# payakorn/InteriorPointMethod

Measured on AMD Instinct MI355X. Metric: IPM iterations/sec (m=4096,n=8192 dense LP), higher is better.
Workload: dtype f64; 1 GPU; dense synthetic LP m=4096 n=8192 fp64, seed 0, start x=s=1 y=0 (BASELINE.json configs[1]); replicas per GPU

## Files before the change

interiorpointmethod_amd/csrc/ff_schedule.h:

```cpp
#pragma once
#include <stdint.h>
#include <stdio.h>
#include <stdlib.h>

#include <math.h>

#include <algorithm>
#include <limits>
#include <queue>
#include <set>
#include <string>
#include <vector>

namespace ipm {

struct FFItem {
    unsigned char type;
    unsigned char i, c;
    unsigned char q;
    union {
        struct { unsigned char j0, j1, flags, seq; } t;
        struct { unsigned short s0, s1; } f;
    };
};
enum { FF_F = 0, FF_T = 1, FF_D = 2 };
enum { FF_INIT = 1, FF_ADD_BASE = 2, FF_PANEL = 4, FF_SIG_DIAG = 8 };
constexpr int FF_MAX_NBLK = 96;

#if defined(__HIPCC__)
#define FF_HD __host__ __device__
#else
#define FF_HD
#endif
FF_HD inline int ff_tile(int i, int c) { return i * (i + 1) / 2 + c; }

struct FFWords {
    static constexpr unsigned ticket = 0;
    static constexpr unsigned role = 3;
    static constexpr unsigned maxbits = 8;
    static constexpr unsigned dcount = 10;
    static constexpr unsigned dbg = 24;
    static constexpr unsigned dbg_end = 32;
    static constexpr unsigned fcount = 32;
    size_t tprog;
    size_t lfinal;
    size_t dready;
    size_t potrfdone;
    size_t count;
    FF_HD explicit FFWords(int nblk) {
        const size_t ntile = (size_t)nblk * ((size_t)nblk + 1) / 2;
        tprog = fcount + ntile; lfinal = tprog + ntile; dready = lfinal + (size_t)nblk; potrfdone = dready + (size_t)nblk;
        count = potrfdone + (size_t)nblk;
    }
    FF_HD static const unsigned* base_of_dbg(const unsigned* dbg_words) { return dbg_words - dbg; }
};

struct FFModel {
    double f_over = 6.1, f_stage = 4.02;
    double f_stage_half = 2.1;
    double t_over = 7.0, t_col = 15.9;
    double t_rmw = 1.0, t_panel = 18.3;
    double t_base = 2.3;
    double d_item = 130.0;
    double gap = 0.8, handoff = 1.0;
    double potrf = 36.8, cpanel = 7.3, cupdate = 7.3;
    int batch = 4;
    int tail = 2;
    double stagger = 0.3;
    int nstages = 512;
    int q_last = 0;
};

struct FFSchedule {
    std::vector<FFItem> items;
    std::vector<int> tile_items;
    std::vector<int> tile_q;
    double makespan_us = 0.0;
    double form_end_us = 0.0;
};

inline int ff_limit(int i, int c) { return (i == c) ? (c > 0 ? c - 1 : 0) : c; }
inline bool ff_needs_panel(int i, int c) { return i > c + 1; }

inline void ff_build_schedule(int nblk, int Q, int W, const FFModel& M_in, FFSchedule& out, int Qmax = 0) {
    if (Qmax < Q) Qmax = Q;
    const double INF = std::numeric_limits<double>::infinity();
    const int ntile = nblk * (nblk + 1) / 2;
    FFModel Mx = M_in;
    if (const char* e = getenv("IPM_FF_BATCH")) Mx.batch = std::max(1, atoi(e));
    if (const char* e = getenv("IPM_FF_TAIL")) Mx.tail = std::max(1, atoi(e));
    if (const char* e = getenv("IPM_FF_STAGGER")) Mx.stagger = std::min(0.9, std::max(0.0, atof(e)));
    if (const char* e = getenv("IPM_FF_Q_LAST")) Mx.q_last = std::max(0, atoi(e));
    if (const char* e = getenv("IPM_FF_MODEL")) {
        std::string spec(e);
        size_t p0 = 0;
        while (p0 < spec.size()) {
            size_t p1 = spec.find(',', p0); if (p1 == std::string::npos) p1 = spec.size();
            const std::string kv = spec.substr(p0, p1 - p0);
            const size_t eq = kv.find('=');
            if (eq != std::string::npos) {
                const std::string k = kv.substr(0, eq); const double v = atof(kv.c_str() + eq + 1);
                struct { const char* n; double* p; } tab[] = {{"f_over", &Mx.f_over}, {"f_stage", &Mx.f_stage}, {"f_stage_half", &Mx.f_stage_half}, {"t_over", &Mx.t_over}, {"t_col", &Mx.t_col},
                    {"t_rmw", &Mx.t_rmw}, {"t_panel", &Mx.t_panel}, {"t_base", &Mx.t_base}, {"d_item", &Mx.d_item}, {"potrf", &Mx.potrf},
                    {"cpanel", &Mx.cpanel}, {"cupdate", &Mx.cupdate}, {"handoff", &Mx.handoff}, {"gap", &Mx.gap}};
                for (auto& t : tab) if (k == t.n) *t.p = v;
            }
            p0 = p1 + 1;
        }
    }
    const FFModel& M = Mx;
    enum Kind { K_F, K_T, K_D, K_POTRF, K_CPANEL, K_CUPDATE };
    struct Node {
        Kind kind; int i = 0, c = 0, q = 0, j0 = 0, j1 = 0, flags = 0, seq = 0, s0 = 0, s1 = 0;
        double dur = 0.0, bl = 0.0, est = 0.0, fin = 0.0;
        int npred = 0, left = 0;
        std::vector<int> succ;
    };
    std::vector<Node> nd;
    nd.reserve((size_t)ntile * 6 + 4 * (size_t)nblk);
    auto add = [&](Kind k, double dur) { Node x; x.kind = k; x.dur = dur; x.fin = INF; nd.push_back(x); return (int)nd.size() - 1; };
    auto edge = [&](int a, int b) { nd[(size_t)a].succ.push_back(b); nd[(size_t)b].npred++; };
    std::vector<int> potrf((size_t)nblk), cpan, cupd;
    for (int k = 0; k < nblk; ++k) { potrf[(size_t)k] = add(K_POTRF, M.potrf + M.handoff); nd.back().i = k; }
    cpan.resize((size_t)nblk - 1); cupd.resize((size_t)nblk - 1);
    for (int k = 0; k + 1 < nblk; ++k) { cpan[(size_t)k] = add(K_CPANEL, M.cpanel + M.handoff); nd.back().i = k; }
    for (int k = 0; k + 1 < nblk; ++k) { cupd[(size_t)k] = add(K_CUPDATE, M.cupdate + M.handoff); nd.back().i = k; }
    for (int k = 0; k + 1 < nblk; ++k) { edge(potrf[(size_t)k], cpan[(size_t)k]); edge(cpan[(size_t)k], cupd[(size_t)k]); edge(cupd[(size_t)k], potrf[(size_t)k + 1]); }
    std::vector<std::vector<int>> titems((size_t)ntile);
    std::vector<int> lprod((size_t)ntile, -1);
    for (int i = 0; i < nblk; ++i)
        for (int c = 0; c <= i; ++c) {
            const int lim = ff_limit(i, c);
            const bool pan = ff_needs_panel(i, c);
            std::vector<std::pair<int, int>> cuts;
            const int nb_end = std::max(0, lim - M.tail);
            int j = 0;
            while (j + M.batch <= nb_end) { cuts.emplace_back(j, j + M.batch); j += M.batch; }
            if (j < nb_end) { cuts.emplace_back(j, nb_end); j = nb_end; }
            while (j < lim) { cuts.emplace_back(j, j + 1); ++j; }
            if (cuts.empty()) cuts.emplace_back(0, 0);
            std::vector<int>& ids = titems[(size_t)ff_tile(i, c)];
            for (size_t s = 0; s < cuts.size(); ++s) {
                const bool last = s + 1 == cuts.size();
                const int id = add(K_T, M.t_over + M.t_col * (cuts[s].second - cuts[s].first) + (s ? M.t_rmw : 0.0) + ((last && pan) ? M.t_panel : 0.0) + M.handoff + M.gap);
                Node& x = nd[(size_t)id];
                x.i = i; x.c = c; x.j0 = cuts[s].first; x.j1 = cuts[s].second; x.seq = (int)s + 1;
                x.flags = (s == 0 ? FF_INIT : 0) | ((last && pan) ? FF_PANEL : 0) | ((last && i == 0 && c == 0) ? FF_SIG_DIAG : 0);
                if (s) edge(ids.back(), id);
                ids.push_back(id);
            }
            if (pan) lprod[(size_t)ff_tile(i, c)] = ids.back();
        }
    for (int k = 0; k + 1 < nblk; ++k) {
        lprod[(size_t)ff_tile(k + 1, k)] = cpan[(size_t)k];
        edge(titems[(size_t)ff_tile(k + 1, k)].back(), cpan[(size_t)k]);
        edge(titems[(size_t)ff_tile(k + 1, k + 1)].back(), cupd[(size_t)k]);
    }
    edge(titems[0].back(), potrf[0]);
    for (int t = 0; t < ntile; ++t)
        for (int id : titems[(size_t)t]) {
            const int i = nd[(size_t)id].i, c = nd[(size_t)id].c, j1 = nd[(size_t)id].j1;
            if (j1 > nd[(size_t)id].j0) {
                edge(lprod[(size_t)ff_tile(i, j1 - 1)], id);
                if (c != i) edge(lprod[(size_t)ff_tile(c, j1 - 1)], id);
            }
            if (nd[(size_t)id].flags & FF_PANEL) edge(potrf[(size_t)c], id);
        }
    std::vector<int> base_item((size_t)ntile);
    for (int t = 0; t < ntile; ++t) { const std::vector<int>& ids = titems[(size_t)t]; base_item[(size_t)t] = ids.size() == 1 ? ids[0] : ids[ids.size() - 2]; }
    std::vector<int> fch;
    out.tile_q.assign((size_t)ntile, 0);
    {
        int npairs = 0;
        for (int i = 0; i < nblk; i += 2)
            for (int c = 0; c <= std::min(i + 1, nblk - 1); ++c) {
                int q = (M.q_last > 0 && i + 2 >= nblk) ? M.q_last : Q;
                q = std::max(1, std::min(std::min(q, Qmax), M.nstages));
                const double phi = std::fmod(npairs * 0.381966, 1.0);
                ++npairs;
                std::vector<int> cut((size_t)q + 1, 0);
                double tot = 0.0, acc = 0.0;
                std::vector<double> len((size_t)q);
                for (int k = 0; k < q; ++k) { len[(size_t)k] = 1.0 + M.stagger * (2.0 * std::fmod((double)k / q + phi, 1.0) - 1.0); tot += len[(size_t)k]; }
                for (int k = 0; k < q; ++k) { acc += len[(size_t)k]; cut[(size_t)k + 1] = (int)(M.nstages * acc / tot + 0.5); }
                cut[(size_t)q] = M.nstages;
                for (int k = 0; k < q; ++k) {
                    const bool half = c > i || i + 1 >= nblk;
                    const int id = add(K_F, M.f_over + (half ? M.f_stage_half : M.f_stage) * (cut[(size_t)k + 1] - cut[(size_t)k]) + M.gap);
                    Node& x = nd[(size_t)id];
                    x.i = i; x.c = c; x.q = k; x.s0 = cut[(size_t)k]; x.s1 = cut[(size_t)k + 1];
                    fch.push_back(id);
                    for (int r = i; r <= i + 1; ++r)
                        if (r >= c && r < nblk) { edge(id, base_item[(size_t)ff_tile(r, c)]); out.tile_q[(size_t)ff_tile(r, c)]++; }
                }
            }
    }
    for (int t = 0; t < ntile; ++t) { Node& x = nd[(size_t)base_item[(size_t)t]]; x.flags |= FF_ADD_BASE; x.dur += M.t_base * out.tile_q[(size_t)t]; }
    std::vector<int> ditems;
    for (int i = 0; i < nblk; ++i) { const int id = add(K_D, M.d_item + M.gap); nd[(size_t)id].i = i; edge(id, potrf[0]); ditems.push_back(id); }
    const int N = (int)nd.size();
    {
        std::vector<int> order, indeg((size_t)N), stack;
        order.reserve((size_t)N);
        for (int u = 0; u < N; ++u) { indeg[(size_t)u] = nd[(size_t)u].npred; if (!indeg[(size_t)u]) stack.push_back(u); }
        while (!stack.empty()) {
            const int u = stack.back(); stack.pop_back(); order.push_back(u);
            for (int v : nd[(size_t)u].succ) if (--indeg[(size_t)v] == 0) stack.push_back(v);
        }
        if ((int)order.size() != N) { out.items.clear(); return; }
        for (size_t k = order.size(); k-- > 0;) {
            Node& x = nd[(size_t)order[k]];
            double b = 0.0;
            for (int v : x.succ) b = std::max(b, nd[(size_t)v].bl);
            x.bl = x.dur + b;
        }
    }
    typedef std::pair<double, int> PI;
    std::priority_queue<PI, std::vector<PI>, std::greater<PI>> avail_F;
    std::set<PI> avail_T;
    for (int id : fch) avail_F.push(PI(-nd[(size_t)id].bl, id));
    for (int u = 0; u < N; ++u) nd[(size_t)u].left = nd[(size_t)u].npred;
    std::vector<int> rel;
    auto release = [&](int u0) {
        rel.clear(); rel.push_back(u0);
        while (!rel.empty()) {
            const int u = rel.back(); rel.pop_back();
            for (int v : nd[(size_t)u].succ) {
                Node& y = nd[(size_t)v];
                y.est = std::max(y.est, nd[(size_t)u].fin);
                if (--y.left == 0) {
                    if (y.kind == K_T) avail_T.insert(PI(-y.bl, v));
                    else if (y.kind != K_F && y.kind != K_D) {
                        y.fin = y.est + y.dur;
                        rel.push_back(v);
                    }
                }
            }
        }
    };
    for (int t = 0; t < ntile; ++t) { const int id = titems[(size_t)t][0]; if (nd[(size_t)id].left == 0) avail_T.insert(PI(-nd[(size_t)id].bl, id)); }
    typedef std::pair<double, int> Ev;
    std::priority_queue<Ev, std::vector<Ev>, std::greater<Ev>> free_at;
    for (int w = 0; w < W; ++w) free_at.push(Ev(0.0, w));
    out.items.clear();
    size_t nT = 0, doneT = 0, nextD = 0;
    for (int t = 0; t < ntile; ++t) nT += titems[(size_t)t].size();
    std::vector<int> order_out;
    int guard = 0;
    while (doneT < nT || !avail_F.empty() || nextD < ditems.size()) {
        const Ev ev = free_at.top(); free_at.pop();
        const double t = ev.first;
        if (nextD < ditems.size()) {
            const int v = ditems[nextD++];
            nd[(size_t)v].fin = t + nd[(size_t)v].dur;
            order_out.push_back(v); release(v);
            free_at.push(Ev(nd[(size_t)v].fin, ev.second));
            continue;
        }
        int pick = -1;
        for (const PI& p : avail_T) if (nd[(size_t)p.second].est <= t) { pick = p.second; break; }
        if (pick >= 0 && !avail_F.empty() && -avail_F.top().first > nd[(size_t)pick].bl) pick = -1;
        if (pick < 0 && !avail_F.empty()) {
            const int v = avail_F.top().second; avail_F.pop();
            nd[(size_t)v].fin = t + nd[(size_t)v].dur;
            out.form_end_us = std::max(out.form_end_us, nd[(size_t)v].fin);
            order_out.push_back(v); release(v);
            free_at.push(Ev(nd[(size_t)v].fin, ev.second));
            continue;
        }
        if (pick < 0) {
            if (avail_T.empty()) {
                if (++guard > 64 * W * nblk) break;
                free_at.push(Ev(t + 5.0, ev.second));
                continue;
            }
            double best = INF;
            for (const PI& p : avail_T) if (nd[(size_t)p.second].est < best) { best = nd[(size_t)p.second].est; pick = p.second; }
        }
        Node& x = nd[(size_t)pick];
        avail_T.erase(PI(-x.bl, pick));
        x.fin = std::max(t, x.est) + x.dur;
        order_out.push_back(pick); ++doneT;
        release(pick);
        free_at.push(Ev(x.fin, ev.second));
    }
    out.tile_items.assign((size_t)ntile, 0);
    for (int t = 0; t < ntile; ++t) out.tile_items[(size_t)t] = (int)titems[(size_t)t].size();
    out.makespan_us = 0.0;
    for (int v : order_out) {
        const Node& x = nd[(size_t)v];
        FFItem it{};
        it.i = (unsigned char)x.i; it.c = (unsigned char)x.c;
        if (x.kind == K_F) { it.type = FF_F; it.q = (unsigned char)x.q; it.f.s0 = (unsigned short)x.s0; it.f.s1 = (unsigned short)x.s1; }
        else if (x.kind == K_D) { it.type = FF_D; }
        else { it.type = FF_T; it.t.j0 = (unsigned char)x.j0; it.t.j1 = (unsigned char)x.j1; it.t.flags = (unsigned char)x.flags; it.t.seq = (unsigned char)x.seq; }
        out.items.push_back(it);
    }
    for (int k = 0; k < nblk; ++k) out.makespan_us = std::max(out.makespan_us, nd[(size_t)potrf[(size_t)k]].fin);
}

}
```

interiorpointmethod_amd/csrc/form_factor.h:

```cpp
#pragma once
#include <hip/hip_runtime.h>
#include <stdint.h>

#include "ff_schedule.h"
#include "gemm_nt_f64.h"
#include "handoff.h"
#include "potrf_f64.h"

namespace ipm {

constexpr int FF_THREADS = 512;
constexpr int FF_BK = 32, FF_LDT = FF_BK + 2;
constexpr int FF_OP = 128 * FF_LDT;
constexpr int FF_LDS_DOUBLES = 4 * FF_OP;

struct FFArgs {
    const double* A; int64_t lda;
    const double* d;
    double* B; int64_t ldb;
    const double* invD;
    double* slab;
    const FFItem* items; int nitems;
    unsigned* ticket;
    unsigned* fcount;
    unsigned* tprog;
    unsigned* lfinal;
    unsigned* dready;
    const unsigned* potrfdone;
    unsigned* timeout;
    unsigned* dbg;
    unsigned dbg_words;
    long long* prof;
    long long* trace;
    const int* done;
    int nblk, Q, nstages;
    int m;
    const int* tile_q;
    unsigned long long* maxbits;
    unsigned* dcount;
};

__device__ __forceinline__ void ff_wait_ge(const unsigned* p, unsigned v, unsigned* timeout, unsigned* dbg = nullptr, unsigned item = 0,
                                           unsigned kind = 0, unsigned nw = 0) {
    (void)handoff_wait<2, false>([=] { return handoff_load(p) >= v; }, {timeout, dbg}, [=] {
        handoff_record_ge(dbg, item, kind, v, p);
        const unsigned* live = FFWords::base_of_dbg(dbg);
        unsigned* snap = const_cast<unsigned*>(live) + nw;
        for (unsigned w = 0; w < nw; ++w) snap[w] = handoff_load(live + w);
    });
}

constexpr int FF_BASE_DEPTH = 4;

template <bool SCALE, bool SRC_REGS>
__device__ __forceinline__ void ff_gemm(const double* __restrict__ Pg, int64_t ldp, const double* __restrict__ Qg, int64_t ldq,
                                        const double* __restrict__ w, int ns, double* lds, f64x4 (&acc)[4][2],
                                        const f64x4 (*src)[2]) {
    const int tid = threadIdx.x, lane = tid & 63;
    const int wave = __builtin_amdgcn_readfirstlane(tid >> 6);
    const int wm = wave >> 2, wn = wave & 3;
    const int fr = lane & 15, fk = lane >> 4;
    double* Ps = lds;
    double* Qs = lds + 2 * FF_OP;
    const int ch = tid & 15, r0 = tid >> 4;
    const double* pP = SRC_REGS ? nullptr : Pg + (int64_t)r0 * ldp + ch * 2;
    const double* pQ = Qg + (int64_t)r0 * ldq + ch * 2;
    f64x2 pr[4], qr[4], wr;
    auto load_stage = [&](int s) {
        if (SCALE) wr = *reinterpret_cast<const f64x2*>(w + (int64_t)s * FF_BK + ch * 2);
#pragma unroll
        for (int u = 0; u < 4; ++u) qr[u] = *reinterpret_cast<const f64x2*>(pQ + (int64_t)u * 32 * ldq + (int64_t)s * FF_BK);
        if (!SRC_REGS) {
#pragma unroll
            for (int u = 0; u < 4; ++u) pr[u] = *reinterpret_cast<const f64x2*>(pP + (int64_t)u * 32 * ldp + (int64_t)s * FF_BK);
        }
    };
    auto store_stage = [&](int s, int buf) {
#pragma unroll
        for (int u = 0; u < 4; ++u) {
            f64x2 v = qr[u];
            if (SCALE) { v.x *= wr.x; v.y *= wr.y; }
            *reinterpret_cast<f64x2*>(Qs + buf * FF_OP + (r0 + 32 * u) * FF_LDT + ch * 2) = v;
        }
        if (!SRC_REGS) {
#pragma unroll
            for (int u = 0; u < 4; ++u) *reinterpret_cast<f64x2*>(Ps + buf * FF_OP + (r0 + 32 * u) * FF_LDT + ch * 2) = pr[u];
        } else if (wn == s) {
#pragma unroll
            for (int i = 0; i < 4; ++i)
#pragma unroll
                for (int j = 0; j < 2; ++j)
#pragma unroll
                    for (int q = 0; q < 4; ++q)
                        Ps[buf * FF_OP + (wm * 64 + i * 16 + fk + 4 * q) * FF_LDT + j * 16 + fr] = src[i][j][q];
        }
    };
    load_stage(0);
    store_stage(0, 0);
    __syncthreads();
    for (int s = 0; s < ns; ++s) {
        const int buf = s & 1;
        if (s + 1 < ns) load_stage(s + 1);
        const double* pa = Ps + buf * FF_OP + (wm * 64 + fr) * FF_LDT + fk;
        const double* qb = Qs + buf * FF_OP + (wn * 32 + fr) * FF_LDT + fk;
#pragma unroll
        for (int kk = 0; kk < FF_BK / 4; ++kk) {
            double a[4], b[2];
#pragma unroll
            for (int i = 0; i < 4; ++i) a[i] = pa[i * 16 * FF_LDT + kk * 4];
#pragma unroll
            for (int j = 0; j < 2; ++j) b[j] = qb[j * 16 * FF_LDT + kk * 4];
#pragma unroll
            for (int i = 0; i < 4; ++i)
#pragma unroll
                for (int j = 0; j < 2; ++j) acc[i][j] = __builtin_amdgcn_mfma_f64_16x16x4f64(a[i], b[j], acc[i][j], 0, 0, 0);
        }
        if (s + 1 < ns) store_stage(s + 1, buf ^ 1);
        __syncthreads();
    }
}

template <bool SCALE, bool HEAD>
__device__ __forceinline__ void ff_gemm_pipe(const double* __restrict__ Pg, int64_t ldp, const double* __restrict__ Qg, int64_t ldq,
                                             const double* __restrict__ w, int ns, double* lds, f64x4 (&acc)[4][2]) {
    const int tid = threadIdx.x, lane = tid & 63;
    const int wave = __builtin_amdgcn_readfirstlane(tid >> 6);
    const int wm = wave >> 2, wn = wave & 3;
    const int fr = lane & 15, fk = lane >> 4;
    double* Ps = lds;
    double* Qs = lds + 2 * FF_OP;
    const int ch = tid & 15, r0 = tid >> 4;
    const double* pP = Pg + (int64_t)r0 * ldp + ch * 2;
    const double* pQ = Qg + (int64_t)r0 * ldq + ch * 2;
    f64x2 pr[4], qr[4], wr;
    auto issue_loads = [&](int s) {
        if (SCALE) wr = *reinterpret_cast<const f64x2*>(w + (int64_t)s * FF_BK + ch * 2);
#pragma unroll
        for (int u = 0; u < 4; ++u) qr[u] = *reinterpret_cast<const f64x2*>(pQ + (int64_t)u * 32 * ldq + (int64_t)s * FF_BK);
#pragma unroll
        for (int u = 0; u < 4; ++u) pr[u] = *reinterpret_cast<const f64x2*>(pP + (int64_t)u * 32 * ldp + (int64_t)s * FF_BK);
    };
    const int st_off = r0 * FF_LDT + ch * 2;
    auto store_q = [&](int buf, int u) {
        f64x2 v = qr[u];
        if (SCALE) { v.x *= wr.x; v.y *= wr.y; }
        *reinterpret_cast<f64x2*>(Qs + buf * FF_OP + u * 32 * FF_LDT + st_off) = v;
    };
    auto store_p = [&](int buf, int u) { *reinterpret_cast<f64x2*>(Ps + buf * FF_OP + u * 32 * FF_LDT + st_off) = pr[u]; };
    const int fa_off = (wm * 64 + fr) * FF_LDT + fk, fb_off = (wn * 32 + fr) * FF_LDT + fk;
    double fa[2][4], fb[2][2];
    auto read_frags = [&](int set, int buf, int kk) {
        const double* pa = Ps + buf * FF_OP + fa_off + kk * 4;
        const double* qb = Qs + buf * FF_OP + fb_off + kk * 4;
#pragma unroll
        for (int i = 0; i < 4; ++i) fa[set][i] = pa[i * 16 * FF_LDT];
#pragma unroll
        for (int j = 0; j < 2; ++j) fb[set][j] = qb[j * 16 * FF_LDT];
    };
    auto mfma8 = [&](int set) {
#pragma unroll
        for (int i = 0; i < 4; ++i)
#pragma unroll
            for (int j = 0; j < 2; ++j) acc[i][j] = __builtin_amdgcn_mfma_f64_16x16x4f64(fa[set][i], fb[set][j], acc[i][j], 0, 0, 0);
    };
    auto mfma_row = [&](int set, int i) {
#pragma unroll
        for (int j = 0; j < 2; ++j) acc[i][j] = __builtin_amdgcn_mfma_f64_16x16x4f64(fa[set][i], fb[set][j], acc[i][j], 0, 0, 0);
    };
    issue_loads(0);
#pragma unroll
    for (int u = 0; u < 4; ++u) { store_q(0, u); store_p(0, u); }
    __syncthreads();
    if (HEAD) issue_loads(min(1, ns - 1));
    else if (1 < ns) issue_loads(1);
    read_frags(0, 0, 0);
    for (int s = 0; s < ns; ++s) {
        const int buf = s & 1;
        const bool more = HEAD || s + 1 < ns;
#pragma unroll
        for (int kk = 0; kk < 6; ++kk) {
            read_frags((kk + 1) & 1, buf, kk + 1);
            __builtin_amdgcn_sched_barrier(0);
            mfma8(kk & 1);
            __builtin_amdgcn_sched_barrier(0);
        }
        read_frags(1, buf, 7);
        __builtin_amdgcn_sched_barrier(0);
#pragma unroll
        for (int i = 0; i < 4; ++i) {
#pragma unroll
            for (int j = 0; j < 2; ++j) acc[i][j] = __builtin_amdgcn_mfma_f64_16x16x4f64(fa[0][i], fb[0][j], acc[i][j], 0, 0, 0);
            if (more) { store_q(buf ^ 1, i); store_p(buf ^ 1, i); }
            __builtin_amdgcn_sched_barrier(0);
        }
        __syncthreads();
        if constexpr (HEAD) {
            mfma_row(1, 0);
            __builtin_amdgcn_sched_barrier(0);
            issue_loads(min(s + 2, ns - 1));
            __builtin_amdgcn_sched_barrier(0);
            mfma_row(1, 1);
            __builtin_amdgcn_sched_barrier(0);
            read_frags(0, buf ^ 1, 0);
            __builtin_amdgcn_sched_barrier(0);
            mfma_row(1, 2);
            mfma_row(1, 3);
            __builtin_amdgcn_sched_barrier(0);
        } else {
            if (s + 2 < ns) issue_loads(s + 2);
            if (more) read_frags(0, buf ^ 1, 0);
            __builtin_amdgcn_sched_barrier(0);
            mfma8(1);
            __builtin_amdgcn_sched_barrier(0);
        }
    }
    __syncthreads();
}

constexpr int FF_PBK = 16, FF_PLDT = FF_PBK + 2;
constexpr int FF_POP_P = 256 * FF_PLDT, FF_POP_Q = 128 * FF_PLDT;
static_assert(2 * (FF_POP_P + FF_POP_Q) <= FF_LDS_DOUBLES, "pair engine LDS");

template <bool HEAD, bool HALF = false>
__device__ __forceinline__ void ff_gemm_pair(const double* __restrict__ P0, const double* __restrict__ P1, const double* __restrict__ Qg,
                                             int64_t ld, const double* __restrict__ w, int ns, double* lds, f64x4 (&acc)[4][4], int lh = 0) {
    static_assert(HEAD || !HALF, "the half-live engine exists on the MFMA-first schedule only");
    constexpr int NP = HALF ? 2 : 4;
    const int tid = threadIdx.x, lane = tid & 63;
    const int wave = __builtin_amdgcn_readfirstlane(tid >> 6);
    const int wm = wave >> 1, wn = wave & 1;
    const int fr = lane & 15, fk = lane >> 4;
    double* Ps = lds;
    double* Qs = lds + 2 * FF_POP_P;
    const int ch = tid & 7, r0 = tid >> 3;
    const double* pP0 = P0 + (int64_t)r0 * ld + ch * 2;
    const double* pP1 = HALF ? nullptr : P1 + (int64_t)r0 * ld + ch * 2;
    const double* pQ = Qg + (int64_t)r0 * ld + ch * 2;
    f64x2 pr[NP], qr[2], wr;
    auto issue_loads = [&](int s) {
        wr = *reinterpret_cast<const f64x2*>(w + (int64_t)s * FF_PBK + ch * 2);
#pragma unroll
        for (int u = 0; u < 2; ++u) qr[u] = *reinterpret_cast<const f64x2*>(pQ + (int64_t)u * 64 * ld + (int64_t)s * FF_PBK);
#pragma unroll
        for (int u = 0; u < 2; ++u) pr[u] = *reinterpret_cast<const f64x2*>(pP0 + (int64_t)u * 64 * ld + (int64_t)s * FF_PBK);
        if constexpr (!HALF) {
#pragma unroll
            for (int u = 0; u < 2; ++u) pr[2 + u] = *reinterpret_cast<const f64x2*>(pP1 + (int64_t)u * 64 * ld + (int64_t)s * FF_PBK);
        }
    };
    const int st_off = r0 * FF_PLDT + ch * 2;
    auto store_q = [&](int buf, int u) {
        f64x2 v = qr[u];
        v.x *= wr.x; v.y *= wr.y;
        *reinterpret_cast<f64x2*>(Qs + buf * FF_POP_Q + u * 64 * FF_PLDT + st_off) = v;
    };
    const int st_off_p = HALF ? st_off + lh * 128 * FF_PLDT : st_off;
    auto store_p = [&](int buf, int u) { *reinterpret_cast<f64x2*>(Ps + buf * FF_POP_P + u * 64 * FF_PLDT + st_off_p) = pr[u]; };
    const int fa_off = (wm * 64 + fr) * FF_PLDT + fk, fb_off = (wn * 64 + fr) * FF_PLDT + fk;
    double fa[2][4], fb[2][4];
    auto read_frags = [&](int set, int buf, int kk) {
        const double* pa = Ps + buf * FF_POP_P + fa_off + kk * 4;
        const double* qb = Qs + buf * FF_POP_Q + fb_off + kk * 4;
#pragma unroll
        for (int i = 0; i < 4; ++i) fa[set][i] = pa[i * 16 * FF_PLDT];
#pragma unroll
        for (int j = 0; j < 4; ++j) fb[set][j] = qb[j * 16 * FF_PLDT];
    };
    auto mfma16 = [&](int set) {
#pragma unroll
        for (int i = 0; i < 4; ++i)
#pragma unroll
            for (int j = 0; j < 4; ++j) acc[i][j] = __builtin_amdgcn_mfma_f64_16x16x4f64(fa[set][i], fb[set][j], acc[i][j], 0, 0, 0);
    };
    auto mfma_row = [&](int set, int i) {
#pragma unroll
        for (int j = 0; j < 4; ++j) acc[i][j] = __builtin_amdgcn_mfma_f64_16x16x4f64(fa[set][i], fb[set][j], acc[i][j], 0, 0, 0);
    };
    issue_loads(0);
#pragma unroll
    for (int u = 0; u < 2; ++u) store_q(0, u);
#pragma unroll
    for (int u = 0; u < NP; ++u) store_p(0, u);
    __syncthreads();
    if (HEAD) issue_loads(min(1, ns - 1));
    else if (1 < ns) issue_loads(1);
    if (HALF && (wm >> 1) != lh) {
        for (int s = 0; s < ns; ++s) {
            const int buf = s & 1;
#pragma unroll
            for (int u = 0; u < 2; ++u) { store_q(buf ^ 1, u); store_p(buf ^ 1, u); }
            __syncthreads();
            issue_loads(min(s + 2, ns - 1));
        }
        __syncthreads();
        return;
    }
    read_frags(0, 0, 0);
    for (int s = 0; s < ns; ++s) {
        const int buf = s & 1;
        const bool more = HEAD || s + 1 < ns;
        read_frags(1, buf, 1);
        __builtin_amdgcn_sched_barrier(0);
        mfma16(0);
        __builtin_amdgcn_sched_barrier(0);
        read_frags(0, buf, 2);
        __builtin_amdgcn_sched_barrier(0);
        mfma16(1);
        __builtin_amdgcn_sched_barrier(0);
        read_frags(1, buf, 3);
        __builtin_amdgcn_sched_barrier(0);
#pragma unroll
        for (int i = 0; i < 4; ++i) {
#pragma unroll
            for (int j = 0; j < 4; ++j) acc[i][j] = __builtin_amdgcn_mfma_f64_16x16x4f64(fa[0][i], fb[0][j], acc[i][j], 0, 0, 0);
            if (more) { if (i < 2) store_q(buf ^ 1, i); if (i < NP) store_p(buf ^ 1, i); }
            __builtin_amdgcn_sched_barrier(0);
        }
        __syncthreads();
        if constexpr (HEAD) {
            mfma_row(1, 0);
            __builtin_amdgcn_sched_barrier(0);
            issue_loads(min(s + 2, ns - 1));
            __builtin_amdgcn_sched_barrier(0);
            mfma_row(1, 1);
            __builtin_amdgcn_sched_barrier(0);
            read_frags(0, buf ^ 1, 0);
            __builtin_amdgcn_sched_barrier(0);
            mfma_row(1, 2);
            mfma_row(1, 3);
            __builtin_amdgcn_sched_barrier(0);
        } else {
            if (s + 2 < ns) issue_loads(s + 2);
            if (more) read_frags(0, buf ^ 1, 0);
            __builtin_amdgcn_sched_barrier(0);
            mfma16(1);
            __builtin_amdgcn_sched_barrier(0);
        }
    }
    __syncthreads();
}


struct FFChain {
    double* B; int64_t ldb; double* invD;
    const unsigned long long* maxbits; const unsigned* dcount; double* maxdiag_out;
    const unsigned* dready; unsigned* potrfdone;
    unsigned* timeout; unsigned* dbg; long long* trace;
    double eps, big, shift_rel;
    int* fixed; const int* done;
    int nblk, m;
};

__device__ __forceinline__ void ff_chain_role(const FFChain& c, double* lds) {
    static_assert(NB * WLD + NB + 2 <= FF_LDS_DOUBLES, "chain role LDS");
    double* W = lds;
    double* dinv_s = lds + NB * WLD;
    double* maxdiag_p = dinv_s + NB;
    const int tid = threadIdx.x;
    if (tid == 0) {
        ff_wait_ge(c.dcount, (unsigned)c.nblk, c.timeout, c.dbg, 9000u, HK_DCOUNT, 0);
        handoff_acquire();
        const double mx = __longlong_as_double((long long)__hip_atomic_load(c.maxbits, __ATOMIC_RELAXED, __HIP_MEMORY_SCOPE_AGENT));
        *maxdiag_p = mx;
        *c.maxdiag_out = mx;
    }
    __syncthreads();
    for (int k = 0; k < c.nblk; ++k) {
        PotrfDiag a;
        a.Bkk = c.B + (int64_t)k * NB * (c.ldb + 1); a.ld = c.ldb;
        a.inv = c.invD + (int64_t)k * NB * NB;
        a.maxdiag = maxdiag_p; a.eps = c.eps; a.big = c.big; a.shift_rel = c.shift_rel;
        a.fixed = c.fixed; a.done = nullptr; a.stamps = nullptr;
        a.wait_on = c.dready + k; a.wait_count = 4u; a.signal = c.potrfdone + k; a.timeout = c.timeout; a.dbg = c.dbg; a.dbg_tag = (unsigned)k;
        a.trace = c.trace ? c.trace + 12 * (size_t)k : nullptr;
        const int real = c.m - k * NB;
        a.nt = (c.shift_rel != 0.0 || real >= NB) ? NB / 16 : (real + 15) / 16 < 1 ? 1 : (real + 15) / 16;
        a.rows = real;
        potrf_diag_body<false>(a, W, dinv_s);
        __syncthreads();
    }
}

struct FFCrit {
    double* B; int64_t ldb; const double* invD;
    const unsigned* tprog; const int* tile_items;
    const unsigned* potrfdone; unsigned* lfinal; unsigned* dready;
    unsigned* timeout; unsigned* dbg; long long* trace;
    const int* done;
    int nblk;
};
constexpr int FF_CRIT_WGS = 4;

__device__ __forceinline__ void ff_crit_role(const FFCrit& c, const int strip, double* lds) {
    static_assert(2 * (32 + 128) * (32 + 2) <= FF_LDS_DOUBLES, "critical role LDS");
    const int tid = threadIdx.x;
    GemmNT g;
    g.w = nullptr; g.M = 128; g.N = 128; g.K = 128; g.lower = 0; g.unit_diag_from = -1; g.done = nullptr;
    g.n_direct = FF_CRIT_WGS; g.split_p = 1; g.chunk_stages = 128 / 32; g.slab = nullptr; g.tile_offset = 0; g.tile_order = nullptr;
    g.sP = g.sQ = g.sC = 0; g.batch = 1; g.sP2 = g.sQ2 = g.sC2 = 0; g.batch2 = 1;
    g.wait_on = nullptr; g.wait_count = 0; g.timeout = nullptr; g.dbg = nullptr; g.dbg_tag = 0; g.trace = nullptr;
    for (int k = 0; k + 1 < c.nblk; ++k) {
        double* panel = c.B + (int64_t)(k + 1) * 128 * c.ldb + (int64_t)k * 128;
        long long* tr = (c.trace && strip == 0 && tid == 0) ? c.trace + 12 * (size_t)k : nullptr;
        if (tr) tr[4] = (long long)wall_clock64();
        if (tid == 0) {
            const int t = ff_tile(k + 1, k);
            ff_wait_ge(c.tprog + t, (unsigned)c.tile_items[t], c.timeout, c.dbg, 1000u + (unsigned)k, HK_GEMM, 0);
            ff_wait_ge(c.potrfdone + k, 1u, c.timeout, c.dbg, 1000u + (unsigned)k, HK_GEMM, 0);
            handoff_acquire();
        }
        __syncthreads();
        if (tr) tr[5] = (long long)wall_clock64();
        g.P = panel; g.ldp = c.ldb; g.Q = c.invD + (int64_t)k * 128 * 128; g.ldq = 128;
        g.C = panel; g.ldc = c.ldb; g.alpha = 1.0; g.beta = 0.0; g.signal = c.lfinal + (k + 1);
        gemm_nt_body<32, 128, 32, 1, 8, false>(g, strip, 0, 0, lds);
        if (tr) { tr[6] = (long long)wall_clock64(); tr[8] = tr[6]; }
        if (tid == 0) {
            const int t = ff_tile(k + 1, k + 1);
            ff_wait_ge(c.lfinal + (k + 1), 4u * (unsigned)(k + 1), c.timeout, c.dbg, 2000u + (unsigned)k, HK_GEMM, 0);
            ff_wait_ge(c.tprog + t, (unsigned)c.tile_items[t], c.timeout, c.dbg, 2000u + (unsigned)k, HK_GEMM, 0);
            handoff_acquire();
        }
        __syncthreads();
        if (tr) tr[9] = (long long)wall_clock64();
        g.P = panel; g.ldp = c.ldb; g.Q = panel; g.ldq = c.ldb;
        g.C = c.B + (int64_t)(k + 1) * 128 * (c.ldb + 1); g.ldc = c.ldb; g.alpha = -1.0; g.beta = 1.0; g.signal = c.dready + (k + 1);
        gemm_nt_body<32, 128, 32, 1, 8, false>(g, strip, 0, 0, lds);
        if (tr) tr[10] = (long long)wall_clock64();
        __syncthreads();
    }
}

enum { FFP_TICKET = 0, FFP_FGEMM, FFP_FSTORE, FFP_TWAIT, FFP_TGEMM, FFP_TBASE, FFP_PWAIT, FFP_PGEMM, FFP_TSTORE, FFP_NF, FFP_NT, FFP_TOTAL };
#define FF_PROF(slot) do { if (TRACE && g.prof && tid == 0) { const long long t_ = __builtin_amdgcn_s_memtime(); g.prof[(size_t)blockIdx.x * 16 + (slot)] += t_ - tprev; tprev = t_; } } while (0)
#define FF_TRACE(slot) do { if (TRACE && g.trace && tid == 0) g.trace[(size_t)n * 4 + (slot)] = (long long)wall_clock64(); } while (0)

struct FFRoles { FFChain chain; FFCrit crit; unsigned* role; };

template <bool TRACE, bool HEAD>
__device__ __forceinline__ void form_factor_body(const FFArgs& g, const FFRoles& r) {
    __shared__ __attribute__((aligned(16))) double lds[FF_LDS_DOUBLES];
    __shared__ unsigned ticket_s;
    if (threadIdx.x == 0) ticket_s = __hip_atomic_fetch_add(r.role, 1u, __ATOMIC_RELAXED, __HIP_MEMORY_SCOPE_AGENT);
    __syncthreads();
    const unsigned role = ticket_s;
    __syncthreads();
    if (role == 0u) { ff_chain_role(r.chain, lds); return; }
    if (role <= (unsigned)FF_CRIT_WGS) { ff_crit_role(r.crit, (int)role - 1, lds); return; }
    const int tid = threadIdx.x, lane = tid & 63;
    const int wave = __builtin_amdgcn_readfirstlane(tid >> 6);
    const int wm = wave >> 2, wn = wave & 3;
    const int fr = lane & 15, fk = lane >> 4;
    const int er = wm * 64 + fk, ec = wn * 32 + fr;

    long long tprev = (TRACE && g.prof) ? __builtin_amdgcn_s_memtime() : 0;
    const long long tstart = tprev;
    for (;;) {
        constexpr unsigned SEL_EXIT = 0xffffffffu;
        if (tid == 0) {
            const unsigned n0 = __hip_atomic_fetch_add(g.ticket, 1u, __ATOMIC_RELAXED, __HIP_MEMORY_SCOPE_AGENT);
            ticket_s = n0 < (unsigned)g.nitems ? n0 : SEL_EXIT;
        }
        __syncthreads();
        const unsigned n = ticket_s;
        __syncthreads();
        if (n == SEL_EXIT) { if (TRACE && g.prof && tid == 0) g.prof[(size_t)blockIdx.x * 16 + FFP_TOTAL] = __builtin_amdgcn_s_memtime() - tstart; return; }
        const FFItem it = g.items[n];
        FF_PROF(FFP_TICKET);
        FF_TRACE(0);
        if (TRACE && g.trace && tid == 0) g.trace[(size_t)n * 4 + 3] = (long long)blockIdx.x;
        const int ti = it.i, tc = it.c;
        const int tile = ff_tile(ti, tc);
        if (it.type == FF_D) {
            double mx = 0.0;
            const int ncols = g.nstages * FF_PBK;
            for (int rr = wave; rr < 128; rr += 8) {
                const int row = ti * 128 + rr;
                if (row >= g.m) break;
                const double* a = g.A + (int64_t)row * g.lda;
                double s0 = 0.0, s1 = 0.0, s2 = 0.0, s3 = 0.0;
                int kq = lane * 2;
                for (; kq + 384 < ncols; kq += 512) {
                    const f64x2 a0 = *reinterpret_cast<const f64x2*>(a + kq), a1 = *reinterpret_cast<const f64x2*>(a + kq + 128);
                    const f64x2 a2 = *reinterpret_cast<const f64x2*>(a + kq + 256), a3 = *reinterpret_cast<const f64x2*>(a + kq + 384);
                    const f64x2 d0 = *reinterpret_cast<const f64x2*>(g.d + kq), d1 = *reinterpret_cast<const f64x2*>(g.d + kq + 128);
                    const f64x2 d2 = *reinterpret_cast<const f64x2*>(g.d + kq + 256), d3 = *reinterpret_cast<const f64x2*>(g.d + kq + 384);
                    s0 = __builtin_fma(a0.x * a0.x, d0.x, s0); s0 = __builtin_fma(a0.y * a0.y, d0.y, s0);
                    s1 = __builtin_fma(a1.x * a1.x, d1.x, s1); s1 = __builtin_fma(a1.y * a1.y, d1.y, s1);
                    s2 = __builtin_fma(a2.x * a2.x, d2.x, s2); s2 = __builtin_fma(a2.y * a2.y, d2.y, s2);
                    s3 = __builtin_fma(a3.x * a3.x, d3.x, s3); s3 = __builtin_fma(a3.y * a3.y, d3.y, s3);
                }
                for (; kq < ncols; kq += 128) {
                    const f64x2 va = *reinterpret_cast<const f64x2*>(a + kq);
                    const f64x2 vd = *reinterpret_cast<const f64x2*>(g.d + kq);
                    s0 = __builtin_fma(va.x * va.x, vd.x, s0);
                    s0 = __builtin_fma(va.y * va.y, vd.y, s0);
                }
                double sacc = (s0 + s1) + (s2 + s3);
#pragma unroll
                for (int o = 32; o > 0; o >>= 1) sacc += __shfl_xor(sacc, o, 64);
                mx = (sacc > mx) ? sacc : mx;
            }
            if (lane == 0) atomicMax(g.maxbits, (unsigned long long)__double_as_longlong(mx));
            handoff_publish_begin();
            if (tid == 0) __hip_atomic_fetch_add(g.dcount, 1u, __ATOMIC_RELAXED, __HIP_MEMORY_SCOPE_AGENT);
            FF_TRACE(2);
            continue;
        }
        if (it.type == FF_F) {
            const bool up = ti >= tc, lo = ti + 1 < g.nblk;
            const int s0 = it.f.s0, s1 = min(g.nstages, (int)it.f.s1);
            f64x4 pacc[4][4];
#pragma unroll
            for (int i = 0; i < 4; ++i)
#pragma unroll
                for (int j = 0; j < 4; ++j) pacc[i][j] = (f64x4){0.0, 0.0, 0.0, 0.0};
            const int r_up = up ? ti : ti + 1, r_lo = lo ? ti + 1 : ti;
            if (s1 > s0) {
                if (HEAD && !(up && lo))
                    ff_gemm_pair<HEAD, HEAD>(g.A + (int64_t)r_up * 128 * g.lda + (int64_t)s0 * FF_PBK, nullptr, g.A + (int64_t)tc * 128 * g.lda + (int64_t)s0 * FF_PBK,
                                             g.lda, g.d + (int64_t)s0 * FF_PBK, s1 - s0, lds, pacc, up ? 0 : 1);
                else
                    ff_gemm_pair<HEAD>(g.A + (int64_t)r_up * 128 * g.lda + (int64_t)s0 * FF_PBK, g.A + (int64_t)r_lo * 128 * g.lda + (int64_t)s0 * FF_PBK,
                                       g.A + (int64_t)tc * 128 * g.lda + (int64_t)s0 * FF_PBK, g.lda, g.d + (int64_t)s0 * FF_PBK, s1 - s0, lds, pacc);
            }
            FF_PROF(FFP_FGEMM);
            {
                const int pm = wave >> 1, pn = wave & 1;
                const int half = pm >> 1;
                if (half == 0 ? up : lo) {
                    const int tl = ff_tile(ti + half, tc);
                    double* sb = g.slab + ((size_t)tl * g.Q + it.q) * (128 * 128) + (size_t)((pm & 1) * 2 + pn) * 4096 + lane * 2;
#pragma unroll
                    for (int i = 0; i < 4; ++i)
#pragma unroll
                        for (int j = 0; j < 4; ++j)
#pragma unroll
                            for (int hq = 0; hq < 2; ++hq)
                                *reinterpret_cast<f64x2*>(sb + ((i * 4 + j) * 2 + hq) * 128) = (f64x2){pacc[i][j][2 * hq], pacc[i][j][2 * hq + 1]};
                }
            }
            handoff_publish_begin();
            if (tid == 0) {
                if (up) __hip_atomic_fetch_add(g.fcount + ff_tile(ti, tc), 1u, __ATOMIC_RELAXED, __HIP_MEMORY_SCOPE_AGENT);
                if (lo) __hip_atomic_fetch_add(g.fcount + ff_tile(ti + 1, tc), 1u, __ATOMIC_RELAXED, __HIP_MEMORY_SCOPE_AGENT);
                if (TRACE && g.prof) g.prof[(size_t)blockIdx.x * 16 + FFP_NF] += 1;
            }
            FF_PROF(FFP_FSTORE);
            FF_TRACE(2);
            continue;
        }

        f64x4 acc[4][2];
#pragma unroll
        for (int i = 0; i < 4; ++i)
#pragma unroll
            for (int j = 0; j < 2; ++j) acc[i][j] = (f64x4){0.0, 0.0, 0.0, 0.0};
        const int j0 = it.t.j0, j1 = it.t.j1;
        const int flags = it.t.flags, seq = it.t.seq;
        int qn_v = 0;
        if (HEAD && (flags & FF_ADD_BASE)) qn_v = g.tile_q[tile];
        if (tid == 0) {
            if (flags & FF_ADD_BASE) ff_wait_ge(g.fcount + tile, (unsigned)g.tile_q[tile], g.timeout, g.dbg, n, HK_FCOUNT, g.dbg_words);
            if (!(flags & FF_INIT)) ff_wait_ge(g.tprog + tile, (unsigned)seq - 1u, g.timeout, g.dbg, n, HK_TPROG, g.dbg_words);
            if (j1 > j0) {
                ff_wait_ge(g.lfinal + ti, 4u * (unsigned)j1, g.timeout, g.dbg, n, HK_LFINAL_ROW, g.dbg_words);
                if (tc != ti) ff_wait_ge(g.lfinal + tc, 4u * (unsigned)j1, g.timeout, g.dbg, n, HK_LFINAL_COL, g.dbg_words);
            }
            handoff_acquire();
        }
        __syncthreads();
        const int qn_s = __builtin_amdgcn_readfirstlane(qn_v);
        FF_PROF(FFP_TWAIT);
        FF_TRACE(1);
        if (j1 > j0)
            ff_gemm_pipe<false, HEAD>(g.B + (int64_t)ti * 128 * g.ldb + (int64_t)j0 * 128, g.ldb,
                                g.B + (int64_t)tc * 128 * g.ldb + (int64_t)j0 * 128, g.ldb, nullptr, (j1 - j0) * (128 / FF_BK), lds, acc);
        FF_PROF(FFP_TGEMM);
        double* bt = g.B + ((int64_t)ti * 128 + er) * g.ldb + (int64_t)tc * 128 + ec;
        f64x4 val[4][2];
#pragma unroll
        for (int i = 0; i < 4; ++i)
#pragma unroll
            for (int j = 0; j < 2; ++j) val[i][j] = (f64x4){0.0, 0.0, 0.0, 0.0};
        if (!(flags & FF_INIT)) {
#pragma unroll
            for (int i = 0; i < 4; ++i)
#pragma unroll
                for (int j = 0; j < 2; ++j)
#pragma unroll
                    for (int q = 0; q < 4; ++q) val[i][j][q] = bt[(int64_t)(i * 16 + 4 * q) * g.ldb + j * 16];
        }
        if constexpr (HEAD) {
            if (flags & FF_ADD_BASE) {
                constexpr int D = FF_BASE_DEPTH;
                static_assert(D == 1 || D == 2 || D == 4, "a ring slot serves the same register groups in every slab");
                const int qn = qn_s;
                unsigned loff = (unsigned)((wm * 2 + (wn >> 1)) * 4096 + (wn & 1) * 512 + lane * 2);
                asm volatile("" : "+v"(loff));
                const double* sb = g.slab + ((size_t)tile * g.Q * (128 * 128) + loff);
                f64x2 ring[D][4];
                auto fill = [&](const double* s, int i) {
#pragma unroll
                    for (int jh = 0; jh < 4; ++jh) ring[i % D][jh] = *reinterpret_cast<const f64x2*>(s + (i * 8 + jh) * 128);
                };
                auto add = [&](int i) {
#pragma unroll
                    for (int jh = 0; jh < 4; ++jh) { val[i][jh >> 1][2 * (jh & 1)] += ring[i % D][jh].x; val[i][jh >> 1][2 * (jh & 1) + 1] += ring[i % D][jh].y; }
                };
#pragma unroll
                for (int i = 0; i < D; ++i) fill(sb, i);
                for (int c = 0; c + 1 < qn; ++c, sb += 128 * 128) {
#pragma unroll
                    for (int i = 0; i < 4; ++i) { add(i); fill(sb + ((i + D) >> 2) * (128 * 128), (i + D) & 3); }
                }
#pragma unroll
                for (int i = 0; i < 4; ++i) { add(i); if (i + D < 4) fill(sb, i + D); }
            }
        } else if (flags & FF_ADD_BASE) {
            const int qn = g.tile_q[tile];
            for (int c = 0; c < qn; ++c) {
                const double* sb = g.slab + ((size_t)tile * g.Q + c) * (128 * 128) + (size_t)(wm * 2 + (wn >> 1)) * 4096 + lane * 2;
#pragma unroll
                for (int i = 0; i < 4; ++i)
#pragma unroll
                    for (int j = 0; j < 2; ++j)
#pragma unroll
                        for (int hq = 0; hq < 2; ++hq) {
                            const f64x2 v = *reinterpret_cast<const f64x2*>(sb + ((i * 4 + (wn & 1) * 2 + j) * 2 + hq) * 128);
                            val[i][j][2 * hq] += v.x; val[i][j][2 * hq + 1] += v.y;
                        }
            }
        }
#pragma unroll
        for (int i = 0; i < 4; ++i)
#pragma unroll
            for (int j = 0; j < 2; ++j) val[i][j] -= acc[i][j];
        if (ti == tc && (flags & FF_ADD_BASE)) {
#pragma unroll
            for (int i = 0; i < 4; ++i)
#pragma unroll
                for (int j = 0; j < 2; ++j)
#pragma unroll
                    for (int q = 0; q < 4; ++q) {
                        const int r = er + i * 16 + 4 * q, c = ec + j * 16;
                        if (r == c && ti * 128 + r >= g.m) val[i][j][q] = 1.0;
                    }
        }
        FF_PROF(FFP_TBASE);
        if (flags & FF_PANEL) {
            if (tid == 0) {
                ff_wait_ge(g.potrfdone + tc, 1u, g.timeout, g.dbg, n, HK_POTRFDONE, g.dbg_words);
                handoff_acquire();
            }
            __syncthreads();
            FF_PROF(FFP_PWAIT);
#pragma unroll
            for (int i = 0; i < 4; ++i)
#pragma unroll
                for (int j = 0; j < 2; ++j) acc[i][j] = (f64x4){0.0, 0.0, 0.0, 0.0};
            ff_gemm<false, true>(nullptr, 0, g.invD + (int64_t)tc * 128 * 128, 128, nullptr, 128 / FF_BK, lds, acc, val);
#pragma unroll
            for (int i = 0; i < 4; ++i)
#pragma unroll
                for (int j = 0; j < 2; ++j) val[i][j] = acc[i][j];
            FF_PROF(FFP_PGEMM);
        }
#pragma unroll
        for (int i = 0; i < 4; ++i)
#pragma unroll
            for (int j = 0; j < 2; ++j)
#pragma unroll
                for (int q = 0; q < 4; ++q) bt[(int64_t)(i * 16 + 4 * q) * g.ldb + j * 16] = val[i][j][q];
        handoff_publish_begin();
        if (tid == 0) {
            __hip_atomic_store(g.tprog + tile, (unsigned)seq, __ATOMIC_RELAXED, __HIP_MEMORY_SCOPE_AGENT);
            if (flags & FF_PANEL) __hip_atomic_fetch_add(g.lfinal + ti, 4u, __ATOMIC_RELAXED, __HIP_MEMORY_SCOPE_AGENT);
            if (flags & FF_SIG_DIAG) __hip_atomic_fetch_add(g.dready + ti, 10u, __ATOMIC_RELAXED, __HIP_MEMORY_SCOPE_AGENT);
            if (TRACE && g.prof) g.prof[(size_t)blockIdx.x * 16 + FFP_NT] += 1;
        }
        FF_PROF(FFP_TSTORE);
        FF_TRACE(2);
    }
}

template <bool TRACE>
__global__ __launch_bounds__(FF_THREADS, 2) void form_factor_roles_kernel(FFArgs g, FFRoles r) {
    if (g.done && *g.done) return;
    form_factor_body<TRACE, false>(g, r);
}
template <bool TRACE>
__global__ __launch_bounds__(FF_THREADS, 2) void form_factor_roles_kernel_mfma_first(FFArgs g, FFRoles r) {
    if (g.done && *g.done) return;
    form_factor_body<TRACE, true>(g, r);
}

__global__ __launch_bounds__(64) void ff_gate_kernel(const unsigned* flag, unsigned value, unsigned* timeout, const int* done) {
    if (done && *done) return;
    if (threadIdx.x == 0) {
        ff_wait_ge(flag, value, timeout);
        handoff_acquire<false>();
    }
}

}
```

Baseline: 279.3 iterations/s.

## Exploit triangular inverse-diagonal block in panel product to skip zero MFMA work

Adds a specialized panel product for the HEAD path that stages the whole tile in LDS and multiplies by the triangular inverse diagonal block, issuing MFMAs only over the nonzero triangle. Each wave is given a balanced pair of output column strips (one near the diagonal, one far from it), and the store offsets are remapped to match. The schedule model's panel cost is lowered to reflect the reduced work. This roughly halves the panel GEMM FLOPs, at the cost of more register pressure from the preloaded B fragments and a remapped output layout that could be wrong if the triangle assumption does not hold.

```diff
diff --git a/interiorpointmethod_amd/csrc/ff_schedule.h b/interiorpointmethod_amd/csrc/ff_schedule.h
--- a/interiorpointmethod_amd/csrc/ff_schedule.h
+++ b/interiorpointmethod_amd/csrc/ff_schedule.h
@@ -59,7 +59,7 @@
     double f_over = 6.1, f_stage = 4.02;
     double f_stage_half = 2.1;
     double t_over = 7.0, t_col = 15.9;
-    double t_rmw = 1.0, t_panel = 18.3;
+    double t_rmw = 1.0, t_panel = 12.3;
     double t_base = 2.3;
     double d_item = 130.0;
     double gap = 0.8, handoff = 1.0;
diff --git a/interiorpointmethod_amd/csrc/form_factor.h b/interiorpointmethod_amd/csrc/form_factor.h
--- a/interiorpointmethod_amd/csrc/form_factor.h
+++ b/interiorpointmethod_amd/csrc/form_factor.h
@@ -118,6 +118,74 @@
         if (s + 1 < ns) store_stage(s + 1, buf ^ 1);
         __syncthreads();
     }
+}
+
+constexpr int FF_TLD = 128 + 2;
+static_assert(128 * FF_TLD <= FF_LDS_DOUBLES, "panel product: the whole tile in LDS");
+
+__device__ __forceinline__ void ff_panel_tri(const double* __restrict__ Qg, double* lds, f64x4 (&acc)[4][2], const f64x4 (&src)[4][2]) {
+    int tid = threadIdx.x;
+    asm volatile("" : "+v"(tid));
+    const int lane = tid & 63;
+    const int wave = __builtin_amdgcn_readfirstlane(tid >> 6);
+    const int wm = wave >> 2, wn = wave & 3;
+    const int fr = lane & 15, fk = lane >> 4;
+    const double* q0 = Qg + (wn * 16 + fr) * 128 + fk;
+    const double* q1 = Qg + ((7 - wn) * 16 + fr) * 128 + fk;
+    double b0[16], b1[32];
+    auto load_b0 = [&](int g) {
+#pragma unroll
+        for (int t = 4 * g; t < 4 * g + 4; ++t) b0[t & 15] = q0[4 * t];
+    };
+    auto load_b1 = [&](int g) {
+#pragma unroll
+        for (int t = 4 * g; t < 4 * g + 4; ++t) b1[t] = q1[4 * t];
+    };
+    auto load_b = [&](int g) {
+        if (g < 8 - wn) load_b1(g);
+        if (g < 4 && g <= wn) load_b0(g);
+    };
+    load_b(0);
+    load_b(1);
+#pragma unroll
+    for (int i = 0; i < 4; ++i)
+#pragma unroll
+        for (int j = 0; j < 2; ++j)
+#pragma unroll
+            for (int q = 0; q < 4; ++q) lds[(wm * 64 + i * 16 + fk + 4 * q) * FF_TLD + wn * 32 + j * 16 + fr] = src[i][j][q];
+    __syncthreads();
+#pragma unroll
+    for (int i = 0; i < 4; ++i)
+#pragma unroll
+        for (int j = 0; j < 2; ++j) acc[i][j] = (f64x4){0.0, 0.0, 0.0, 0.0};
+    const double* pa = lds + (wm * 64 + fr) * FF_TLD + fk;
+#pragma unroll
+    for (int g = 0; g < 8; ++g) {
+        if (g + 2 < 8) load_b(g + 2);
+        if (g < 4 && g <= wn) {
+#pragma unroll
+            for (int t = 4 * g; t < 4 * g + 4; ++t) {
+                double a[4];
+#pragma unroll
+                for (int i = 0; i < 4; ++i) a[i] = pa[i * 16 * FF_TLD + 4 * t];
+#pragma unroll
+                for (int i = 0; i < 4; ++i) {
+                    acc[i][0] = __builtin_amdgcn_mfma_f64_16x16x4f64(a[i], b0[t & 15], acc[i][0], 0, 0, 0);
+                    acc[i][1] = __builtin_amdgcn_mfma_f64_16x16x4f64(a[i], b1[t], acc[i][1], 0, 0, 0);
+                }
+            }
+        } else if (g < 8 - wn) {
+#pragma unroll
+            for (int t = 4 * g; t < 4 * g + 4; ++t) {
+                double a[4];
+#pragma unroll
+                for (int i = 0; i < 4; ++i) a[i] = pa[i * 16 * FF_TLD + 4 * t];
+#pragma unroll
+                for (int i = 0; i < 4; ++i) acc[i][1] = __builtin_amdgcn_mfma_f64_16x16x4f64(a[i], b1[t], acc[i][1], 0, 0, 0);
+            }
+        }
+    }
+    __syncthreads();
 }
 
 template <bool SCALE, bool HEAD>
@@ -648,6 +716,7 @@
                     }
         }
         FF_PROF(FFP_TBASE);
+        int cj0 = 0, cj1 = 16;
         if (flags & FF_PANEL) {
             if (tid == 0) {
                 ff_wait_ge(g.potrfdone + tc, 1u, g.timeout, g.dbg, n, HK_POTRFDONE, g.dbg_words);
@@ -655,11 +724,17 @@
             }
             __syncthreads();
             FF_PROF(FFP_PWAIT);
-#pragma unroll
-            for (int i = 0; i < 4; ++i)
-#pragma unroll
-                for (int j = 0; j < 2; ++j) acc[i][j] = (f64x4){0.0, 0.0, 0.0, 0.0};
-            ff_gemm<false, true>(nullptr, 0, g.invD + (int64_t)tc * 128 * 128, 128, nullptr, 128 / FF_BK, lds, acc, val);
+            if constexpr (HEAD) {
+                ff_panel_tri(g.invD + (int64_t)tc * 128 * 128, lds, acc, val);
+                cj0 = -16 * wn;
+                cj1 = 16 * (7 - 3 * wn);
+            } else {
+#pragma unroll
+                for (int i = 0; i < 4; ++i)
+#pragma unroll
+                    for (int j = 0; j < 2; ++j) acc[i][j] = (f64x4){0.0, 0.0, 0.0, 0.0};
+                ff_gemm<false, true>(nullptr, 0, g.invD + (int64_t)tc * 128 * 128, 128, nullptr, 128 / FF_BK, lds, acc, val);
+            }
 #pragma unroll
             for (int i = 0; i < 4; ++i)
 #pragma unroll
@@ -671,7 +746,7 @@
 #pragma unroll
             for (int j = 0; j < 2; ++j)
 #pragma unroll
-                for (int q = 0; q < 4; ++q) bt[(int64_t)(i * 16 + 4 * q) * g.ldb + j * 16] = val[i][j][q];
+                for (int q = 0; q < 4; ++q) bt[(int64_t)(i * 16 + 4 * q) * g.ldb + (HEAD ? (j ? cj1 : cj0) : j * 16)] = val[i][j][q];
         handoff_publish_begin();
         if (tid == 0) {
             __hip_atomic_store(g.tprog + tile, (unsigned)seq, __ATOMIC_RELAXED, __HIP_MEMORY_SCOPE_AGENT);
```

Result: no change. 279.1 iterations/s (-0.1%).
